# mrvollger/rustybam

Hardware: NVIDIA B200
Metric: lifted window-records/s (higher is better)
Workload: dtype u32/u64 (+f32 identities)

## Files before the change

rustybam_b200/csrc/rb_kernels.cu:

```cuda
#include <algorithm>
#include <cstdio>

#include "f32_fmt.cuh"
#include "lift_core.cuh"
#include "rb_kernels.cuh"
#include "rec_core.cuh"
#include "stream_core.cuh"

namespace rb {

__device__ __forceinline__ uint4 ld_nc_v4(const void* p) {
    uint4 r;
    asm volatile("ld.global.nc.L1::no_allocate.v4.u32 {%0,%1,%2,%3}, [%4];" : "=r"(r.x), "=r"(r.y), "=r"(r.z), "=r"(r.w) : "l"(p));
    return r;
}
__device__ __forceinline__ unsigned long long ld_volatile_u64(const unsigned long long* p) {
    unsigned long long v;
    asm volatile("ld.volatile.global.u64 %0, [%1];" : "=l"(v) : "l"(p));
    return v;
}
__device__ __forceinline__ uint32_t ld_volatile_u32(const uint32_t* p) {
    uint32_t v;
    asm volatile("ld.volatile.global.u32 %0, [%1];" : "=r"(v) : "l"(p));
    return v;
}
__device__ __forceinline__ uint4 ld_cg_v4(const void* p) {
    uint4 r;
    asm volatile("ld.global.cg.v4.u32 {%0,%1,%2,%3}, [%4];" : "=r"(r.x), "=r"(r.y), "=r"(r.z), "=r"(r.w) : "l"(p));
    return r;
}
__device__ __forceinline__ void report(unsigned long long* slot, uint64_t key, uint32_t code) {
    atomicMin(slot, (unsigned long long)((key << 8) | code));
}
__device__ __forceinline__ uint32_t nondigit_bytes(uint32_t x) {
    const uint32_t t = x ^ 0x30303030u;
    return (((t & 0x7F7F7F7Fu) + 0x76767676u) | t) & 0x80808080u;
}
__device__ __forceinline__ uint32_t nondigit_count(uint4 c) {
    return __popc(nondigit_bytes(c.x)) + __popc(nondigit_bytes(c.y)) + __popc(nondigit_bytes(c.z)) + __popc(nondigit_bytes(c.w));
}
// ... 50 lines not shown
    }
    if (lane == 0) atomicExch(&state[tile], LB_PRE | (excl + agg));
    return excl;
}

__device__ __forceinline__ void lb_publish(unsigned long long* state, uint64_t tile, unsigned long long agg) {
    atomicExch(&state[tile], (tile == 0 ? LB_PRE : LB_AGG) | agg);
}
__device__ __forceinline__ unsigned long long lb_walk(unsigned long long* state, uint64_t tile, unsigned long long agg) {
    const int lane = threadIdx.x & 31;
    if (tile == 0) return 0;
    unsigned long long excl = 0;
    long long look = (long long)tile - 1;
    for (;;) {
        const long long idx = look - lane;
        unsigned long long s = LB_PRE;
        if (idx >= 0) {
            s = ld_volatile_u64(&state[idx]);
            while ((s >> 62) == 0) { __nanosleep(64); s = ld_volatile_u64(&state[idx]); }
        }
        const unsigned pm = __ballot_sync(0xffffffffu, (s >> 62) == 2);
        const int first = pm ? (__ffs(pm) - 1) : 32;
        unsigned long long v = (lane <= first) ? (s & LB_VAL) : 0ull;
#pragma unroll
        for (int d = 16; d > 0; d >>= 1) v += __shfl_xor_sync(0xffffffffu, v, d);
        excl += v;
        if (pm) break;
        look -= 32;
    }
    if (lane == 0) atomicExch(&state[tile], LB_PRE | (excl + agg));
    return excl;
}

__device__ __noinline__ bool exact_len(const uint8_t* text, uint64_t pos, uint32_t& len, uint32_t& err) {
    long long s = (long long)pos;
    while (text[s - 1] >= '0' && text[s - 1] <= '9') s--;
    if (s == (long long)pos) { err = RE_CIGAR_PARSE; return false; }
    unsigned long long v = 0;
    for (long long k = s; k < (long long)pos; k++) {
        v = v * 10ull + (unsigned long long)(text[k] - '0');
        if (v > 0xFFFFFFFFull) { err = RE_CIGAR_PARSE; return false; }
    }
    if (v > MAX_OP_LEN) { err = RE_UNSUPPORTED; return false; }
    len = (uint32_t)v;
    return true;
}

__device__ __forceinline__ uint32_t smem_u32(const void* p) { return (uint32_t)__cvta_generic_to_shared(p); }
__device__ __forceinline__ void mbar_init(unsigned long long* bar, uint32_t count) {
    asm volatile("mbarrier.init.shared::cta.b64 [%0], %1;" ::"r"(smem_u32(bar)), "r"(count) : "memory");
    asm volatile("fence.mbarrier_init.release.cluster;" ::: "memory");
}
__device__ __forceinline__ void mbar_expect_tx(unsigned long long* bar, uint32_t bytes) {
    asm volatile("mbarrier.arrive.expect_tx.shared::cta.b64 _, [%0], %1;" ::"r"(smem_u32(bar)), "r"(bytes) : "memory");
}
__device__ __forceinline__ void bulk_g2s(void* dst, const void* src, uint32_t bytes, unsigned long long* bar) {
    asm volatile("cp.async.bulk.shared::cluster.global.mbarrier::complete_tx::bytes [%0], [%1], %2, [%3];" ::"r"(smem_u32(dst)),
                 "l"(src), "r"(bytes), "r"(smem_u32(bar))
                 : "memory");
}
__device__ __forceinline__ void fence_proxy_async() { asm volatile("fence.proxy.async.shared::cta;" ::: "memory"); }
__device__ __forceinline__ void bulk_s2g(void* dst, const void* src, uint32_t bytes) {
    asm volatile("cp.async.bulk.global.shared::cta.bulk_group [%0], [%1], %2;" ::"l"(dst), "r"(smem_u32(src)), "r"(bytes) : "memory");
    asm volatile("cp.async.bulk.commit_group;" ::: "memory");
}
__device__ __forceinline__ void bulk_wait_read() { asm volatile("cp.async.bulk.wait_group.read 0;" ::: "memory"); }
__device__ __forceinline__ void mbar_wait(unsigned long long* bar, uint32_t parity) {
    asm volatile(
        "{\n"
        ".reg .pred P1;\n"
        "LAB_WAIT:\n"
        "mbarrier.try_wait.parity.shared::cta.b64 P1, [%0], %1;\n"
        "@P1 bra DONE;\n"
        "bra LAB_WAIT;\n"
        "DONE:\n"
        "}\n" ::"r"(smem_u32(bar)),
        "r"(parity)
        : "memory");
}
__device__ __forceinline__ uint32_t parse4(uint32_t x) {
    x &= 0x0F0F0F0Fu;
    const uint32_t pairs = ((x * 2561u) >> 8) & 0x00FF00FFu;
    return (pairs * 6553601u) >> 16;
}

__global__ void __launch_bounds__(TOK_THREADS)
k_tokenise(const uint8_t* __restrict__ text, uint32_t* __restrict__ ops, unsigned long long* tile_state, unsigned int* ticket,
           ErrSlots err, uint32_t* misc_flags) {
    __shared__ __align__(16) uint8_t s_text[16 + TOK_TILE + 16];
    __shared__ uint16_t s_pos[TOK_TILE / 2];
#if RB_TOK_EARLY_PUBLISH
    __shared__ uint32_t s_opw[TOK_TILE / 2];
#endif
    __shared__ uint8_t s_lut[256];
    __shared__ __align__(8) unsigned long long s_bar;
    __shared__ uint32_t s_warp[TOK_THREADS / 32];
    __shared__ unsigned long long s_base;
    __shared__ unsigned int s_tile;

    const int tid = threadIdx.x, lane = tid & 31, warp = tid >> 5;
    if (tid < 256) s_lut[tid] = (uint8_t)code_of_char((uint32_t)tid);
    if (tid == 0) {
        s_tile = atomicAdd(ticket, 1u);
        mbar_init(&s_bar, 1);
    }
    __syncthreads();
    const uint64_t tile = s_tile;
    const uint64_t tbase = tile * (uint64_t)TOK_TILE;
    if (tid == 0) {
        mbar_expect_tx(&s_bar, 16 + TOK_TILE);
        bulk_g2s(s_text, text + tbase - 16, 16 + TOK_TILE, &s_bar);
    }
    mbar_wait(&s_bar, 0);

    const uint4 c = *reinterpret_cast<const uint4*>(s_text + 16 + tid * 16);
    const uint32_t M = 0x01020408u;
    const uint32_t m16 = ((((nondigit_bytes(c.x) >> 7) * M) >> 24) & 0xFu) | (((((nondigit_bytes(c.y) >> 7) * M) >> 24) & 0xFu) << 4) |
                         (((((nondigit_bytes(c.z) >> 7) * M) >> 24) & 0xFu) << 8) | (((((nondigit_bytes(c.w) >> 7) * M) >> 24) & 0xFu) << 12);
    const uint32_t cnt = __popc(m16);

    uint32_t inc = cnt;
#pragma unroll
    for (int d = 1; d < 32; d <<= 1) {
        const uint32_t t = __shfl_up_sync(0xffffffffu, inc, d);
        if (lane >= d) inc += t;
    }
    if (lane == 31) s_warp[warp] = inc;
    {
        uint32_t mm = m16, k = 0;
        const uint32_t wex = inc - cnt;
        __syncthreads();
        uint32_t wpre = 0, total = 0;
#pragma unroll
        for (int w = 0; w < TOK_THREADS / 32; w++) {
            const uint32_t t = s_warp[w];
            if (w < warp) wpre += t;
            total += t;
        }
#if RB_TOK_EARLY_PUBLISH
        if (tid == 0) lb_publish(tile_state, tile, total);
#else
        if (warp == 0) {
            const unsigned long long ex = lookback_u64(tile_state, tile, total);
            if (lane == 0) s_base = ex;
        }
#endif
        uint32_t idx = wpre + wex;
        while (mm) {
            const uint32_t j = __ffs(mm) - 1;
            mm &= mm - 1;
            s_pos[idx + k] = (uint16_t)(tid * 16 + j);
            k++;
        }
        __syncthreads();
        const uint32_t* s_w = reinterpret_cast<const uint32_t*>(s_text);
        uint32_t seen_codes = 0;
#if !RB_TOK_EARLY_PUBLISH
        const uint64_t base = s_base;
        uint32_t* out_ops = ops + base;
#endif
        for (uint32_t q = tid; q < total; q += TOK_THREADS) {
            const uint32_t e = s_pos[q];
            const uint32_t a = (e + 8) >> 2, sh = ((e + 8) & 3) * 8;
            const uint32_t w0 = s_w[a], w1 = s_w[a + 1], w2 = s_w[a + 2];
            uint32_t lo = __funnelshift_r(w0, w1, sh);
            uint32_t hi = __funnelshift_r(w1, w2, sh);
            uint32_t nd;
            if (q > 0) {
                nd = e - s_pos[q - 1] - 1u;
                nd = nd > 8u ? 8u : nd;
            } else {
                const uint32_t nh = nondigit_bytes(hi), nl = nondigit_bytes(lo);
                nd = nh ? (__clz(nh) >> 3) : (4u + (nl ? (__clz(nl) >> 3) : 4u));
            }
            const uint32_t code = s_lut[s_text[16 + e]];
            uint32_t len;
            if (nd - 1u >= 7u || code == 15u) {
                uint32_t ecode = RE_CIGAR_PARSE;
                len = 0;
                if (code == 15u || !exact_len(text, tbase + e, len, ecode)) { report(err.tok, tbase + e, ecode); len = 0; }
            } else {
                const unsigned long long x = (((unsigned long long)hi << 32) | lo) & (~0ull << (8u * (8u - nd)));
                len = parse4((uint32_t)(x >> 32));
                if (nd > 4u) len += parse4((uint32_t)x) * 10000u;
            }
            seen_codes |= 1u << code;
            const uint32_t word = (len << 4) | (code == 15u ? (uint32_t)OP_P : code);
#if RB_TOK_EARLY_PUBLISH
            s_opw[q] = word;
#else
            out_ops[q] = word;
#endif
        }
        const uint32_t seen_clip = seen_codes & ((1u << OP_S) | (1u << OP_H));
        if (seen_clip) atomicOr(misc_flags, 1u);
#if RB_TOK_EARLY_PUBLISH
        if (warp == 0) {
            const unsigned long long ex = lb_walk(tile_state, tile, total);
            if (lane == 0) s_base = ex;
        }
        __syncthreads();
        uint32_t* out_ops = ops + s_base;
        for (uint32_t q = tid; q < total; q += TOK_THREADS) out_ops[q] = s_opw[q];
#endif
    }
}

__global__ void __launch_bounds__(256)
k_rec_ops(const uint8_t* __restrict__ text, const uint64_t* __restrict__ cigar_off, uint32_t n_rec,
          const unsigned long long* __restrict__ tile_state, uint64_t* __restrict__ op_off, uint32_t* heads, ErrSlots err) {
    const uint32_t r = (blockIdx.x * blockDim.x + threadIdx.x) >> 5;
    const int lane = threadIdx.x & 31;
    if (r > n_rec) return;
    const uint64_t c = cigar_off[r];
    const uint64_t tile = c / TOK_TILE, tbase = tile * (uint64_t)TOK_TILE;
    const uint64_t prefix = tile ? (tile_state[tile - 1] & LB_VAL) : 0ull;
    const uint32_t nfull = (uint32_t)((c - tbase) >> 4), rem = (uint32_t)((c - tbase) & 15u);
    uint32_t cnt = 0;
    for (uint32_t j = lane; j < nfull; j += 32) cnt += nondigit_count(ld_nc_v4(text + tbase + (uint64_t)j * 16u));
    if (lane == 0 && rem) {
        const uint4 x = ld_nc_v4(text + tbase + (uint64_t)nfull * 16u);
        const uint32_t xw[4] = {x.x, x.y, x.z, x.w};
        for (uint32_t j = 0; j < rem; j++) cnt += ((((xw[j >> 2] >> ((j & 3) * 8)) & 0xFFu) - 48u) >= 10u);
    }
#pragma unroll
    for (int d = 16; d > 0; d >>= 1) cnt += __shfl_xor_sync(0xffffffffu, cnt, d);
    if (lane == 0) {
        const uint64_t o = prefix + cnt;
        op_off[r] = o;
        if (r < n_rec) {
            const uint64_t len = cigar_off[r + 1] - c;
            if (len > 0) {
                atomicOr(&heads[o >> 5], 1u << (o & 31u));
                const uint32_t last = text[c + len - 1], first = text[c];
                if ((last - 48u) < 10u) report(err.rec, r, RE_CIGAR_PARSE);
                if ((first - 48u) >= 10u) report(err.rec, r, RE_CIGAR_PARSE);
            }
        }
    }
}

__device__ __forceinline__ uint32_t flip_indel(uint32_t w) {
    const uint32_t c = op_code(w);
    return (c == OP_I || c == OP_D) ? (w ^ 3u) : w;
}
__global__ void __launch_bounds__(256)
k_invert_ops(uint32_t* __restrict__ ops, const uint64_t* __restrict__ op_off, uint32_t n_rec, const uint8_t* __restrict__ strand) {
    const uint64_t k = (uint64_t)blockIdx.x * blockDim.x + threadIdx.x;
    if (n_rec == 0 || k >= op_off[n_rec]) return;
    uint32_t lo = 0, hi = n_rec;
    while (lo < hi) {
        const uint32_t mid = lo + ((hi - lo) >> 1);
        if (op_off[mid] <= k) lo = mid + 1; else hi = mid;
    }
    const uint32_t r = lo - 1;
    const uint64_t a = op_off[r], b = op_off[r + 1];
    if (strand[r] != '-') { ops[k] = flip_indel(ops[k]); return; }
    const uint64_t i = k - a, m = b - 1 - i;
    if (k < m) {
        const uint32_t x = ops[k], y = ops[m];
        ops[k] = flip_indel(y);
// ... 589 lines not shown
#pragma unroll
        for (int k = 0; k < SMP_THREADS / 32; k++) btot = seg_combine(btot, s_warp[k]);
#if RB_SMP2_LB2
        const SegVal ex = lookback_seg2(blk_agg, b, btot);
#else
        const SegVal ex = lookback_seg(blk_state, blk_agg, blk_pre, b, btot);
#endif
        if (lane == 0) s_blk = ex;
    } else {
        for (int k = 0; k < warp; k++) wpre = seg_combine(wpre, s_warp[k]);
    }
    __syncthreads();
    SegVal pre = seg_combine(seg_combine(s_blk, wpre), exl);
    if (h & 1u) pre.c = ctr_zero();
    if (no_subs) pre.c.aux = (pre.c.aux & ~SUB_ABS) | SUB_ABS;
    if (nvalid) samples[chunk * SUBS] = pre.c;
}

constexpr uint32_t TS_NONE = 0xFFFFFFFFu;
__global__ void __launch_bounds__(256)
k_rec_heads(const uint8_t* __restrict__ text, const uint64_t* __restrict__ cigar_off, uint32_t n_rec, uint64_t* __restrict__ head_pos,
            uint32_t* tile_first) {
    const uint32_t r = blockIdx.x * blockDim.x + threadIdx.x;
    if (r >= n_rec) return;
    const uint64_t c = cigar_off[r], e = cigar_off[r + 1];
    uint64_t hp = ~0ull;
    const uint64_t lim = (e - c > 16u) ? c + 16u : e;
    for (uint64_t p = c; p < lim; p++)
        if (((uint32_t)text[p] - 48u) >= 10u) { hp = p; break; }
    head_pos[r] = hp;
    if (hp != ~0ull) atomicMin(&tile_first[hp / TOK_TILE], r);
}

#ifndef RB_TOKSCAN_MINB
#define RB_TOKSCAN_MINB 4
#endif
__global__ void __launch_bounds__(TOK_THREADS, RB_TOKSCAN_MINB)
k_tok_scan(const uint8_t* __restrict__ text, uint32_t* __restrict__ ops, unsigned long long* tile_state, unsigned int* ticket,
           ErrSlots err, uint32_t* misc_flags, const uint32_t* __restrict__ tile_first, const uint64_t* __restrict__ head_pos,
           uint32_t n_rec, Ctr* __restrict__ samples, uint32_t* seg_state, ScanPayload* seg_agg, ScanPayload* seg_pre) {
    __shared__ __align__(16) uint8_t s_text[16 + TOK_TILE + 16];
    __shared__ uint16_t s_pos[TOK_TILE / 2];
    __shared__ uint32_t s_opw[TOK_TILE / 2];
    __shared__ uint32_t s_head[TOK_TILE / 64 + 1];
    __shared__ uint16_t s_excl[TOK_THREADS], s_m16[TOK_THREADS];
    __shared__ uint8_t s_lut[256];
    __shared__ __align__(8) unsigned long long s_bar;
    __shared__ uint32_t s_warp[TOK_THREADS / 32];
    __shared__ SegVal s_wagg[TOK_THREADS / 32];
    __shared__ SegVal s_blk;
    __shared__ unsigned long long s_base;
    __shared__ unsigned int s_tile;
    __shared__ uint32_t s_prev0;

    const int tid = threadIdx.x, lane = tid & 31, warp = tid >> 5;
    if (tid < 256) s_lut[tid] = (uint8_t)code_of_char((uint32_t)tid);
    if (tid < TOK_TILE / 64 + 1) s_head[tid] = 0u;
    if (tid == 0) {
        s_tile = atomicAdd(ticket, 1u);
        mbar_init(&s_bar, 1);
        s_prev0 = 99u;
    }
    __syncthreads();
    const uint64_t tile = s_tile;
    const uint64_t tbase = tile * (uint64_t)TOK_TILE;
    if (tid == 0) {
        mbar_expect_tx(&s_bar, 16 + TOK_TILE);
        bulk_g2s(s_text, text + tbase - 16, 16 + TOK_TILE, &s_bar);
    }
    uint32_t r_first = TS_NONE;
    if (warp == TOK_THREADS / 32 - 1) r_first = tile_first[tile];
    mbar_wait(&s_bar, 0);

    const uint4 c = *reinterpret_cast<const uint4*>(s_text + 16 + tid * 16);
    const uint32_t M = 0x01020408u;
    const uint32_t m16 = ((((nondigit_bytes(c.x) >> 7) * M) >> 24) & 0xFu) | (((((nondigit_bytes(c.y) >> 7) * M) >> 24) & 0xFu) << 4) |
                         (((((nondigit_bytes(c.z) >> 7) * M) >> 24) & 0xFu) << 8) | (((((nondigit_bytes(c.w) >> 7) * M) >> 24) & 0xFu) << 12);
    const uint32_t cnt = __popc(m16);
    uint32_t inc = cnt;
#pragma unroll
    for (int d = 1; d < 32; d <<= 1) {
        const uint32_t t = __shfl_up_sync(0xffffffffu, inc, d);
        if (lane >= d) inc += t;
    }
    if (lane == 31) s_warp[warp] = inc;
    s_m16[tid] = (uint16_t)m16;
    __syncthreads();
    uint32_t wpre = 0, total = 0;
#pragma unroll
    for (int w = 0; w < TOK_THREADS / 32; w++) {
        const uint32_t t = s_warp[w];
        if (w < warp) wpre += t;
        total += t;
    }
    if (warp == 0) {
        const unsigned long long ex = lookback_u64(tile_state, tile, total);
        if (lane == 0) s_base = ex;
    }
    {
        uint32_t mm = m16, k = 0;
        const uint32_t idx = wpre + inc - cnt;
        s_excl[tid] = (uint16_t)idx;
        while (mm) {
            const uint32_t j = __ffs(mm) - 1;
            mm &= mm - 1;
            s_pos[idx + k] = (uint16_t)(tid * 16 + j);
            k++;
        }
    }
    __syncthreads();
    const uint64_t base = s_base;
    if (r_first != TS_NONE) {
        const uint64_t tend = tbase + TOK_TILE;
        for (uint64_t r = (uint64_t)r_first + lane; r < n_rec; r += 32) {
            const uint64_t hp = head_pos[r];
            if (hp == ~0ull) continue;
            if (hp >= tend) break;
            const uint32_t bpos = (uint32_t)(hp - tbase), t = bpos >> 4;
            const uint32_t j = (uint32_t)s_excl[t] + __popc((uint32_t)s_m16[t] & ((1u << (bpos & 15u)) - 1u));
            atomicOr(&s_head[j >> 5], 1u << (j & 31u));
        }
    }
    {
        const uint32_t* s_w = reinterpret_cast<const uint32_t*>(s_text);
        uint32_t seen_codes = 0;
        uint32_t* out_ops = ops + base;
        for (uint32_t q = tid; q < total; q += TOK_THREADS) {
            const uint32_t e = s_pos[q];
            const uint32_t a = (e + 8) >> 2, sh = ((e + 8) & 3) * 8;
            const uint32_t w0 = s_w[a], w1 = s_w[a + 1], w2 = s_w[a + 2];
            uint32_t lo = __funnelshift_r(w0, w1, sh);
            uint32_t hi = __funnelshift_r(w1, w2, sh);
            uint32_t nd;
            if (q > 0) {
                nd = e - s_pos[q - 1] - 1u;
                nd = nd > 8u ? 8u : nd;
            } else {
                const uint32_t nh = nondigit_bytes(hi), nl = nondigit_bytes(lo);
                nd = nh ? (__clz(nh) >> 3) : (4u + (nl ? (__clz(nl) >> 3) : 4u));
                int p = 16 + (int)e - 1;
                while (p >= 0 && ((uint32_t)s_text[p] - 48u) < 10u) p--;
                s_prev0 = (p >= 0) ? (uint32_t)s_lut[s_text[p]] : 99u;
            }
            const uint32_t code = s_lut[s_text[16 + e]];
            uint32_t len;
            if (nd - 1u >= 7u || code == 15u) {
                uint32_t ecode = RE_CIGAR_PARSE;
                len = 0;
                if (code == 15u || !exact_len(text, tbase + e, len, ecode)) { report(err.tok, tbase + e, ecode); len = 0; }
            } else {
                const unsigned long long x = (((unsigned long long)hi << 32) | lo) & (~0ull << (8u * (8u - nd)));
                len = parse4((uint32_t)(x >> 32));
                if (nd > 4u) len += parse4((uint32_t)x) * 10000u;
            }
            seen_codes |= 1u << code;
            const uint32_t word = (len << 4) | (code == 15u ? (uint32_t)OP_P : code);
            out_ops[q] = word;
            s_opw[q] = word;
        }
        const uint32_t seen_clip = seen_codes & ((1u << OP_S) | (1u << OP_H));
        if (seen_clip) atomicOr(misc_flags, 1u);
    }
    __syncthreads();

    const uint32_t off = (uint32_t)(base & 7u);
    const uint32_t ngroups = total ? ((total + off + 7u) >> 3) : 0u;
    const uint32_t per = (ngroups + TOK_THREADS - 1) / TOK_THREADS;
    const uint32_t g0 = (uint32_t)tid * per;
    const int lo_op = (int)(g0 * 8u) - (int)off;
    const uint32_t j_lo = lo_op < 0 ? 0u : (uint32_t)lo_op;
    uint32_t j_hi = (g0 + per) * 8u - off;
    j_hi = j_hi > total ? total : j_hi;
    SegVal mine = seg_identity();
    if (g0 < ngroups) {
        uint32_t slowc = 0;
        uint32_t prev_code = j_lo ? op_code(s_opw[j_lo - 1]) : s_prev0;
        for (uint32_t j = j_lo; j < j_hi; j++) {
            const uint32_t w = s_opw[j];
            const bool head = (s_head[j >> 5] >> (j & 31u)) & 1u;
            if (head) { mine.c = ctr_zero(); slowc = 0; mine.flag = 1u; }
            const uint32_t code = op_code(w), n = op_len(w);
            slowc += ((n - 1u) >= (ACC_BIG - 1u)) | ((!head) & (code == prev_code));
            ctr_add_op(mine.c, w);
            prev_code = code;
        }
        mine.c.aux = (mine.c.aux & AUX_OVF) | (slowc & AUX_CNT);
    }
    SegVal sinc = mine;
#pragma unroll
    for (int d = 1; d < 32; d <<= 1) {
        const SegVal y = seg_shfl(sinc, (lane - d) & 31);
        if (lane >= d) sinc = seg_combine(y, sinc);
    }
    if (lane == 31) s_wagg[warp] = sinc;
    SegVal exl = seg_shfl(sinc, (lane - 1) & 31);
    if (lane == 0) exl = seg_identity();
    __syncthreads();
    SegVal wp = seg_identity();
    if (warp == 0) {
        SegVal btot = seg_identity();
#pragma unroll
        for (int k = 0; k < TOK_THREADS / 32; k++) btot = seg_combine(btot, s_wagg[k]);
#ifdef RB_TS_NOLB
        const SegVal ex = btot;
#else
        const SegVal ex = lookback_seg(seg_state, seg_agg, seg_pre, tile, btot);
#endif
        if (lane == 0) s_blk = ex;
    } else {
        for (int k = 0; k < warp; k++) wp = seg_combine(wp, s_wagg[k]);
    }
    __syncthreads();
    if (g0 >= ngroups) return;
    SegVal pre = seg_combine(seg_combine(s_blk, wp), exl);
    for (uint32_t gi = 0; gi < per && g0 + gi < ngroups; gi++) {
        const int ls = (int)((g0 + gi) * 8u) - (int)off;
        if (gi) {
            const uint32_t a0 = (ls - 8) < 0 ? 0u : (uint32_t)(ls - 8);
            uint32_t slowc = pre.c.aux & AUX_CNT, ovf = pre.c.aux & AUX_OVF;
            uint32_t prev_code = a0 ? op_code(s_opw[a0 - 1]) : s_prev0;
            for (uint32_t j = a0; j < (uint32_t)ls; j++) {
                const uint32_t w = s_opw[j];
                const bool head = (s_head[j >> 5] >> (j & 31u)) & 1u;
                if (head) { pre.c = ctr_zero(); slowc = 0; ovf = 0; }
                const uint32_t code = op_code(w), n = op_len(w);
                slowc += ((n - 1u) >= (ACC_BIG - 1u)) | ((!head) & (code == prev_code));
                pre.c.aux = 0;
                ctr_add_op(pre.c, w);
                ovf |= pre.c.aux & AUX_OVF;
                prev_code = code;
            }
            pre.c.aux = ovf | (slowc & AUX_CNT);
        }
        if (ls < 0 || (uint32_t)ls >= total) continue;
        Ctr out = pre.c;
// ... 1700 lines not shown
    put_op(out_text + body_of(r) + pos, op_len(w), op_code(w));
}

static size_t samples2_smem() { return (size_t)(SMP_THREADS * SAMPLE + 9 * SMP_THREADS) * sizeof(uint32_t); }
static size_t scan_lift_smem(bool lift) {
    return (size_t)(SMP_THREADS * (SAMPLE + 1) + 9 * SMP_THREADS + (lift ? 2 * SL_WCAP : 0)) * sizeof(uint32_t);
}
int init_kernel_attrs() {
    cudaError_t e = cudaFuncSetAttribute(k_scan_lift<true>, cudaFuncAttributeMaxDynamicSharedMemorySize, (int)scan_lift_smem(true));
    if (e == cudaSuccess) e = cudaFuncSetAttribute(k_scan_lift<false>, cudaFuncAttributeMaxDynamicSharedMemorySize, (int)scan_lift_smem(false));
    if (e == cudaSuccess) e = cudaFuncSetAttribute(k_samples2<true>, cudaFuncAttributeMaxDynamicSharedMemorySize, (int)samples2_smem());
    if (e == cudaSuccess) e = cudaFuncSetAttribute(k_samples2<false>, cudaFuncAttributeMaxDynamicSharedMemorySize, (int)samples2_smem());
    if (e == cudaSuccess) e = cudaFuncSetAttribute(k_samples2<false, true>, cudaFuncAttributeMaxDynamicSharedMemorySize, (int)samples2_smem());
    if (e == cudaSuccess) e = cudaFuncSetAttribute(k_serialise, cudaFuncAttributeMaxDynamicSharedMemorySize, SER_CAP);
    if (e == cudaSuccess) e = cudaFuncSetAttribute(k_emit<false>, cudaFuncAttributeMaxDynamicSharedMemorySize, EMIT_DYN_BYTES);
    if (e == cudaSuccess) e = cudaFuncSetAttribute(k_emit<true>, cudaFuncAttributeMaxDynamicSharedMemorySize, EMIT_DYN_BYTES);
    return e == cudaSuccess ? 0 : -1;
}
__global__ void k_add_u64(unsigned long long* __restrict__ p, uint64_t n, unsigned long long delta) {
    const uint64_t i = (uint64_t)blockIdx.x * blockDim.x + threadIdx.x;
    if (i < n) p[i] += delta;
}
void launch_add_u64(uint64_t* p, uint64_t n, uint64_t delta, cudaStream_t s) {
    if (n == 0 || delta == 0) return;
    k_add_u64<<<(unsigned)((n + 255) / 256), 256, 0, s>>>(reinterpret_cast<unsigned long long*>(p), n, delta);
}
void launch_whole_text(const uint32_t* ops, const uint64_t* op_off, uint32_t n_rec, const RecInfo* recs, const Ctr* samples,
                       const uint64_t* line_off, uint8_t* out_text, uint64_t n_ops_bound, cudaStream_t s) {
    if (n_rec == 0 || n_ops_bound == 0 || out_text == nullptr) return;
    const uint64_t chunks = (n_ops_bound + SAMPLE - 1) / SAMPLE;
    k_whole_text<<<(unsigned)((chunks + WT_THREADS / 32 - 1) / (WT_THREADS / 32)), WT_THREADS, 0, s>>>(ops, op_off, n_rec, recs, samples,
                                                                                                    line_off, out_text);
}
void launch_tokenise(const uint8_t* text, uint64_t n_tiles, uint32_t* ops, unsigned long long* tile_state, unsigned int* ticket,
                     ErrSlots err, uint32_t* misc_flags, cudaStream_t s) {
    if (n_tiles == 0) return;
    k_tokenise<<<(unsigned)n_tiles, TOK_THREADS, 0, s>>>(text, ops, tile_state, ticket, err, misc_flags);
}
void launch_tok_scan(const uint8_t* text, uint64_t n_tiles, const uint64_t* cigar_off, uint32_t n_rec, uint32_t* ops,
                     unsigned long long* tile_state, unsigned int* ticket, ErrSlots err, uint32_t* misc_flags, uint32_t* tile_first,
                     uint64_t* head_pos, Ctr* samples, uint32_t* seg_state, ScanPayload* seg_agg, ScanPayload* seg_pre, cudaStream_t s) {
    if (n_tiles == 0) return;
    if (n_rec) k_rec_heads<<<(n_rec + 255) / 256, 256, 0, s>>>(text, cigar_off, n_rec, head_pos, tile_first);
    k_tok_scan<<<(unsigned)n_tiles, TOK_THREADS, 0, s>>>(text, ops, tile_state, ticket, err, misc_flags, tile_first, head_pos, n_rec,
                                                         samples, seg_state, seg_agg, seg_pre);
}
void launch_rec_ops(const uint8_t* text, const uint64_t* cigar_off, uint32_t n_rec, const unsigned long long* tile_state,
                    uint64_t* op_off, uint32_t* heads, ErrSlots err, cudaStream_t s) {
    const uint64_t warps = (uint64_t)n_rec + 1;
    k_rec_ops<<<(unsigned)((warps * 32 + 255) / 256), 256, 0, s>>>(text, cigar_off, n_rec, tile_state, op_off, heads, err);
}
void launch_scan_lift(bool lift, const uint32_t* ops, const uint64_t* n_ops_dev, uint64_t n_ops_bound, const uint32_t* heads,
                      Ctr* samples, uint32_t* blk_state, ScanPayload* blk_agg, ScanPayload* blk_pre, unsigned int* ticket,
                      LiftArgs la, cudaStream_t s, bool no_subs) {
    const uint64_t blocks = (n_ops_bound + SMP_OPS - 1) / SMP_OPS;
    if (blocks == 0) return;
    if (lift)
        k_scan_lift<true><<<(unsigned)blocks, SMP_THREADS, scan_lift_smem(true), s>>>(ops, n_ops_dev, heads, samples, blk_state, blk_agg,
                                                                                      blk_pre, ticket, la);
    else if (getenv("RB_OLD_SAMPLES"))
        k_scan_lift<false><<<(unsigned)blocks, SMP_THREADS, scan_lift_smem(false), s>>>(ops, n_ops_dev, heads, samples, blk_state,
                                                                                        blk_agg, blk_pre, ticket, la);
    else if (!getenv("RB_SAMPLES_LOCAL")) {
#if RB_SMP2_LB2
        cudaMemsetAsync(blk_agg, 0, blocks * sizeof(ScanPayload), s);
#endif
        if (no_subs)
            k_samples2<false, true><<<(unsigned)blocks, SMP_THREADS, samples2_smem(), s>>>(ops, n_ops_dev, heads, samples, blk_state, blk_agg, blk_pre,
                                                                                           ticket, 1u);
        else
            k_samples2<false><<<(unsigned)blocks, SMP_THREADS, samples2_smem(), s>>>(ops, n_ops_dev, heads, samples, blk_state, blk_agg, blk_pre, ticket,
                                                                                     0u);
    } else {
        k_samples2<true><<<(unsigned)blocks, SMP_THREADS, samples2_smem(), s>>>(ops, n_ops_dev, heads, samples, blk_state, blk_agg, blk_pre, ticket, 0u);
        k_blk_scan<<<1, 1024, 0, s>>>(n_ops_dev, blk_agg, blk_pre);
        const uint64_t chunks = (n_ops_bound + SAMPLE - 1) / SAMPLE;
        k_smp_fix<<<(unsigned)((chunks + 255) / 256), 256, 0, s>>>(n_ops_dev, blk_pre, samples);
// ... 213 lines not shown
```

rustybam_b200/csrc/rb_kernels.cuh:

```cuda
#pragma once
#include <cuda_runtime.h>

#include "lift_core.cuh"
#include "rb_common.cuh"
#include "trim_core.cuh"

namespace rb {

#ifndef RB_TOK_THREADS
#define RB_TOK_THREADS 256
#endif
constexpr int TOK_THREADS = RB_TOK_THREADS;
#ifndef RB_TOK_EARLY_PUBLISH
#define RB_TOK_EARLY_PUBLISH 1
#endif
constexpr int TOK_TILE = TOK_THREADS * 16;
constexpr int TEXT_FRONT_PAD = 16;
#ifndef RB_SMP_THREADS
#define RB_SMP_THREADS 256
#endif
constexpr int SMP_THREADS = RB_SMP_THREADS;
constexpr int SMP_OPS = SMP_THREADS * (int)SAMPLE;
constexpr int SL_WCAP = 2048;
#ifndef RB_LIFT_THREADS
#define RB_LIFT_THREADS 128
#endif
#ifndef RB_LIFT_CCAP
#define RB_LIFT_CCAP 96
#endif
#ifndef RB_LIFT_MINB
#define RB_LIFT_MINB 6
#endif
#ifndef RB_LIFT_STAGE_SMP
#define RB_LIFT_STAGE_SMP 1
#endif
#ifndef RB_LIFT_CHAIN
#define RB_LIFT_CHAIN 1
#endif
#ifndef RB_SMP2_LB2
#define RB_SMP2_LB2 0
#endif
#ifndef RB_SMP_MINB
#define RB_SMP_MINB 3
#endif
#ifndef RB_EMIT_MINB
#define RB_EMIT_MINB 6
#endif
#ifndef RB_EMIT_STAGE_TEXT
#define RB_EMIT_STAGE_TEXT 0
// ... 30 lines not shown
    const uint32_t* cont_hi;
    const uint32_t* pair_win;
    uint32_t general;
    uint32_t from_record;
};

struct RecInput {
    const uint64_t* cigar_off;
    const uint64_t *q_len, *q_st, *q_en, *t_len, *t_st, *t_en, *mapq;
    const uint8_t* strand;
    const uint32_t *q_id, *t_id;
    const uint64_t* names_off;
    const uint8_t* names;
    uint32_t n_rec;
    uint32_t no_text;
};

struct StatsDev {
    uint32_t *equal, *diff, *ins, *del, *ins_ev, *del_ev, *matches;
    float *id_m, *id_e, *id_a;
};
struct NumDev {
    uint64_t *q_st, *q_en, *t_st, *t_en, *nmatch, *aln_len;
    uint32_t *rec_idx, *win_idx;
};

struct ErrSlots {
    unsigned long long* tok;
    unsigned long long* rec;
};

int init_kernel_attrs();
void launch_add_u64(uint64_t* p, uint64_t n, uint64_t delta, cudaStream_t s);
void launch_tokenise(const uint8_t* text, uint64_t n_tiles, uint32_t* ops, unsigned long long* tile_state,
                     unsigned int* ticket, ErrSlots err, uint32_t* misc_flags, cudaStream_t s);
void launch_tok_scan(const uint8_t* text, uint64_t n_tiles, const uint64_t* cigar_off, uint32_t n_rec, uint32_t* ops,
                     unsigned long long* tile_state, unsigned int* ticket, ErrSlots err, uint32_t* misc_flags, uint32_t* tile_first,
                     uint64_t* head_pos, Ctr* samples, uint32_t* seg_state, ScanPayload* seg_agg, ScanPayload* seg_pre, cudaStream_t s);
void launch_rec_ops(const uint8_t* text, const uint64_t* cigar_off, uint32_t n_rec, const unsigned long long* tile_state,
                    uint64_t* op_off, uint32_t* heads, ErrSlots err, cudaStream_t s);
struct LiftArgs {
    const RecInfo* recs;
    const uint64_t* op_off;
    uint32_t n_rec;
    const uint32_t* rec_rank;
    const uint64_t* pair_off;
    const uint64_t* w_st;
    const uint64_t* w_en;
    HalfS* hs;
    HalfE* he;
};
void launch_scan_lift(bool lift, const uint32_t* ops, const uint64_t* n_ops_dev, uint64_t n_ops_bound, const uint32_t* heads,
                      Ctr* samples, uint32_t* blk_state, ScanPayload* blk_agg, ScanPayload* blk_pre, unsigned int* ticket,
                      LiftArgs la, cudaStream_t s, bool no_subs = false);
void launch_combine(uint64_t n_pairs, const uint64_t* pair_off, const uint32_t* rec_order, uint32_t n_rec, const RecInfo* recs,
                    const uint32_t* ops, WinView win, const uint64_t* names_off, const HalfS* hs, const HalfE* he, PairRes* res,
                    uint32_t* line_len, ErrSlots err, cudaStream_t s);
void launch_invert_ops(uint32_t* ops, const uint64_t* op_off, uint32_t n_rec, const uint8_t* strand, uint64_t n_ops_bound,
                       cudaStream_t s);
void launch_check_clips(const uint32_t* ops, const uint64_t* op_off, uint32_t n_rec, ErrSlots err, cudaStream_t s);
void launch_rec_prep(int mode, RecInput in, const uint64_t* op_off, const uint32_t* ops, const Ctr* samples, WinView win,
                     RecInfo* recs, uint32_t* pair_cnt, StatsDev st, ErrSlots err, cudaStream_t s);
void launch_pair_scan(const uint32_t* pair_cnt, const uint32_t* rec_order, uint32_t n_rec, uint64_t* pair_off, cudaStream_t s);
enum : uint32_t { PLAN_UNIFORM = 1u,
                  PLAN_FAST = 2u };
struct LiftPlan {
    uint32_t k0;
// ... 113 lines not shown
```

rustybam_b200/csrc/rbcuda.cu:

```cuda
#include <algorithm>
#include <chrono>
#include <condition_variable>
#include <cstdarg>
#include <cstdio>
#include <cstdlib>
#include <cstring>
#include <functional>
#include <mutex>
#include <string>
#include <thread>
#include <unordered_map>
#include <vector>

#include <sys/mman.h>

#include "../../include/rbcuda.h"
#include "name_intern.hpp"
#include "paf_parse_core.cuh"
#include "rb_kernels.cuh"
#include "rec_core.cuh"
#include "trim_rounds.hpp"

using namespace rb;

// ... 354 lines not shown
    NumDev d{};
    uint64_t* p = b->out_num.as<uint64_t>();
    d.q_st = p; d.q_en = p + n; d.t_st = p + 2 * n; d.t_en = p + 3 * n; d.nmatch = p + 4 * n; d.aln_len = p + 5 * n;
    d.rec_idx = reinterpret_cast<uint32_t*>(p + 6 * n);
    d.win_idx = d.rec_idx + n;
    return d;
}

bool tok_scan_enabled() {
    static const bool on = getenv("RB_TOKSCAN") != nullptr;
    return on;
}

int run_tok(rb_ctx* ctx, rb_batch* b) {
    cudaStream_t s = ctx->stream;
    uint32_t* sc = ctx->scalars.as<uint32_t>();
    CU(cudaMemsetAsync(sc, 0, 4 * sizeof(uint32_t), s));
    CU(cudaMemsetAsync(sc + SC_ERR_TOK, 0xFF, 4 * sizeof(uint32_t), s));
    CU(cudaMemsetAsync(b->tile_state.p, 0, b->n_tiles * 8, s));
    CU(cudaMemsetAsync(b->heads.p, 0, (b->ops_bound / SAMPLE + 2) * 4, s));
    CU(cudaMemsetAsync(b->blk_state.p, 0, (b->ops_bound / SMP_OPS + 2) * 4, s));
    ErrSlots err{reinterpret_cast<unsigned long long*>(sc + SC_ERR_TOK), reinterpret_cast<unsigned long long*>(sc + SC_ERR_REC)};
    const uint8_t* text = b->text_raw.as<uint8_t>() + TEXT_FRONT_PAD;
    b->have_samples = !b->invert && tok_scan_enabled();
    if (b->have_samples) {
        CU(cudaMemsetAsync(b->tile_first.p, 0xFF, b->n_tiles * 4, s));
        CU(cudaMemsetAsync(b->seg_state.p, 0, b->n_tiles * 4, s));
        KScope k(ctx, "k_tok_scan");
        launch_tok_scan(text, b->n_tiles, b->cigar_off.as<uint64_t>(), b->n_rec, b->ops.as<uint32_t>(), b->tile_state.as<unsigned long long>(),
                        sc + SC_TICKET_TOK, err, sc + SC_MISC, b->tile_first.as<uint32_t>(), b->head_pos.as<uint64_t>(), b->samples.as<Ctr>(),
                        b->seg_state.as<uint32_t>(), b->seg_agg.as<ScanPayload>(), b->seg_pre.as<ScanPayload>(), s);
    } else {
        KScope k(ctx, "k_tokenise");
        launch_tokenise(text, b->n_tiles, b->ops.as<uint32_t>(), b->tile_state.as<unsigned long long>(), sc + SC_TICKET_TOK, err,
                        sc + SC_MISC, s);
    }
    {
        KScope k(ctx, "k_rec_ops");
        launch_rec_ops(text, b->cigar_off.as<uint64_t>(), b->n_rec, b->tile_state.as<unsigned long long>(), b->op_off.as<uint64_t>(),
                       b->heads.as<uint32_t>(), err, s);
    }
    if (b->invert) {
        KScope k(ctx, "k_invert_ops");
        launch_invert_ops(b->ops.as<uint32_t>(), b->op_off.as<uint64_t>(), b->n_rec, b->strand.as<uint8_t>(), b->ops_bound, s);
    }
    CU(cudaGetLastError());
    return RB_OK;
}

int run_scan(rb_ctx* ctx, rb_batch* b, const LiftArgs* la, bool no_subs = false) {
    cudaStream_t s = ctx->stream;
    uint32_t* sc = ctx->scalars.as<uint32_t>();
    if (!la && b->have_samples) return RB_OK;
    {
        KScope k(ctx, la ? "k_scan_lift" : "k_samples");
        launch_scan_lift(la != nullptr, b->ops.as<uint32_t>(), b->op_off.as<uint64_t>() + b->n_rec, b->ops_bound, b->heads.as<uint32_t>(),
                         b->samples.as<Ctr>(), b->blk_state.as<uint32_t>(), b->blk_agg.as<ScanPayload>(), b->blk_pre.as<ScanPayload>(),
                         sc + SC_TICKET_SMP, la ? *la : LiftArgs{}, s, no_subs && !la);
    }
    CU(cudaGetLastError());
    return RB_OK;
}

}

extern "C" {

// ... 2603 lines not shown
```

Measured before the change: 447.6 million.

## Restructure CIGAR tokenizer to per-thread runs with staged vectorized op writes

The tokenise kernel now has each thread handle a 32-byte run instead of 16 bytes, which doubles the tile size. Each thread parses its own delimiters sequentially in registers instead of going through a shared position array and a second strided pass. Parsed words are staged in shared memory and written to global memory with aligned uint4 stores after the lookback. The k_tok_scan kernel is resized to keep its 16 bytes per thread under the larger tile, which changes its block size and min-blocks launch bound. A per-tile cap and a clamp on op_off are added to bound writes when the text ends early. The trade-off is more serial work per thread and fewer, larger tiles.

Result: faster. 478.8 million (median of 6 runs) (+7.0%).

```diff
diff --git a/rustybam_b200/csrc/rb_kernels.cu b/rustybam_b200/csrc/rb_kernels.cu
--- a/rustybam_b200/csrc/rb_kernels.cu
+++ b/rustybam_b200/csrc/rb_kernels.cu
@@ -6,6 +6,7 @@
 #include "rb_kernels.cuh"
 #include "rec_core.cuh"
 #include "stream_core.cuh"
+#include "tok_core.cuh"
 
 namespace rb {
 
@@ -122,18 +123,11 @@
     return excl;
 }
 
-__device__ __noinline__ bool exact_len(const uint8_t* text, uint64_t pos, uint32_t& len, uint32_t& err) {
-    long long s = (long long)pos;
-    while (text[s - 1] >= '0' && text[s - 1] <= '9') s--;
-    if (s == (long long)pos) { err = RE_CIGAR_PARSE; return false; }
-    unsigned long long v = 0;
-    for (long long k = s; k < (long long)pos; k++) {
-        v = v * 10ull + (unsigned long long)(text[k] - '0');
-        if (v > 0xFFFFFFFFull) { err = RE_CIGAR_PARSE; return false; }
-    }
-    if (v > MAX_OP_LEN) { err = RE_UNSUPPORTED; return false; }
-    len = (uint32_t)v;
-    return true;
+__device__ __noinline__ uint32_t tok_rare(const uint8_t* text, uint64_t pos, uint32_t code, unsigned long long* slot) {
+    uint32_t ecode;
+    const uint32_t w = tok_exact(text, pos, code, ecode);
+    if (ecode != RE_OK) report(slot, pos, ecode);
+    return w;
 }
 
 __device__ __forceinline__ uint32_t smem_u32(const void* p) { return (uint32_t)__cvta_generic_to_shared(p); }
@@ -175,13 +169,10 @@
 }
 
 __global__ void __launch_bounds__(TOK_THREADS)
-k_tokenise(const uint8_t* __restrict__ text, uint32_t* __restrict__ ops, unsigned long long* tile_state, unsigned int* ticket,
-           ErrSlots err, uint32_t* misc_flags) {
-    __shared__ __align__(16) uint8_t s_text[16 + TOK_TILE + 16];
-    __shared__ uint16_t s_pos[TOK_TILE / 2];
-#if RB_TOK_EARLY_PUBLISH
-    __shared__ uint32_t s_opw[TOK_TILE / 2];
-#endif
+k_tokenise(const uint8_t* __restrict__ text, uint64_t n_bytes, uint32_t* __restrict__ ops, unsigned long long* tile_state,
+           unsigned int* ticket, ErrSlots err, uint32_t* misc_flags) {
+    __shared__ __align__(16) uint8_t s_text[TOK_HALO + TOK_TILE];
+    __shared__ __align__(16) uint32_t s_opw[TOK_TILE / 2 + 4];
     __shared__ uint8_t s_lut[256];
     __shared__ __align__(8) unsigned long long s_bar;
     __shared__ uint32_t s_warp[TOK_THREADS / 32];
@@ -189,7 +180,7 @@
     __shared__ unsigned int s_tile;
 
     const int tid = threadIdx.x, lane = tid & 31, warp = tid >> 5;
-    if (tid < 256) s_lut[tid] = (uint8_t)code_of_char((uint32_t)tid);
+    for (int c = tid; c < 256; c += TOK_THREADS) s_lut[c] = (uint8_t)tok_code_of_char((uint32_t)c);
     if (tid == 0) {
         s_tile = atomicAdd(ticket, 1u);
         mbar_init(&s_bar, 1);
@@ -198,17 +189,20 @@
     const uint64_t tile = s_tile;
     const uint64_t tbase = tile * (uint64_t)TOK_TILE;
     if (tid == 0) {
-        mbar_expect_tx(&s_bar, 16 + TOK_TILE);
-        bulk_g2s(s_text, text + tbase - 16, 16 + TOK_TILE, &s_bar);
+        mbar_expect_tx(&s_bar, TOK_HALO + TOK_TILE);
+        bulk_g2s(s_text, text + tbase - TOK_HALO, TOK_HALO + TOK_TILE, &s_bar);
     }
     mbar_wait(&s_bar, 0);
 
-    const uint4 c = *reinterpret_cast<const uint4*>(s_text + 16 + tid * 16);
-    const uint32_t M = 0x01020408u;
-    const uint32_t m16 = ((((nondigit_bytes(c.x) >> 7) * M) >> 24) & 0xFu) | (((((nondigit_bytes(c.y) >> 7) * M) >> 24) & 0xFu) << 4) |
-                         (((((nondigit_bytes(c.z) >> 7) * M) >> 24) & 0xFu) << 8) | (((((nondigit_bytes(c.w) >> 7) * M) >> 24) & 0xFu) << 12);
-    const uint32_t cnt = __popc(m16);
-
+    const uint32_t* s_w = reinterpret_cast<const uint32_t*>(s_text);
+    uint32_t w[TOK_RUN / 4];
+#pragma unroll
+    for (int i = 0; i < TOK_RUN / 16; i++) {
+        const uint4 v = *reinterpret_cast<const uint4*>(s_text + TOK_HALO + tid * TOK_RUN + 16 * i);
+        w[4 * i] = v.x; w[4 * i + 1] = v.y; w[4 * i + 2] = v.z; w[4 * i + 3] = v.w;
+    }
+    const tok_mask_t<TOK_RUN> m = tok_run_mask<TOK_RUN>(w);
+    const uint32_t cnt = tok_popc(m);
     uint32_t inc = cnt;
 #pragma unroll
     for (int d = 1; d < 32; d <<= 1) {
@@ -216,84 +210,48 @@
         if (lane >= d) inc += t;
     }
     if (lane == 31) s_warp[warp] = inc;
-    {
-        uint32_t mm = m16, k = 0;
-        const uint32_t wex = inc - cnt;
-        __syncthreads();
-        uint32_t wpre = 0, total = 0;
-#pragma unroll
-        for (int w = 0; w < TOK_THREADS / 32; w++) {
-            const uint32_t t = s_warp[w];
-            if (w < warp) wpre += t;
-            total += t;
-        }
-#if RB_TOK_EARLY_PUBLISH
-        if (tid == 0) lb_publish(tile_state, tile, total);
-#else
-        if (warp == 0) {
-            const unsigned long long ex = lookback_u64(tile_state, tile, total);
-            if (lane == 0) s_base = ex;
-        }
-#endif
-        uint32_t idx = wpre + wex;
-        while (mm) {
-            const uint32_t j = __ffs(mm) - 1;
-            mm &= mm - 1;
-            s_pos[idx + k] = (uint16_t)(tid * 16 + j);
-            k++;
-        }
-        __syncthreads();
-        const uint32_t* s_w = reinterpret_cast<const uint32_t*>(s_text);
-        uint32_t seen_codes = 0;
-#if !RB_TOK_EARLY_PUBLISH
-        const uint64_t base = s_base;
-        uint32_t* out_ops = ops + base;
-#endif
-        for (uint32_t q = tid; q < total; q += TOK_THREADS) {
-            const uint32_t e = s_pos[q];
-            const uint32_t a = (e + 8) >> 2, sh = ((e + 8) & 3) * 8;
-            const uint32_t w0 = s_w[a], w1 = s_w[a + 1], w2 = s_w[a + 2];
-            uint32_t lo = __funnelshift_r(w0, w1, sh);
-            uint32_t hi = __funnelshift_r(w1, w2, sh);
-            uint32_t nd;
-            if (q > 0) {
-                nd = e - s_pos[q - 1] - 1u;
-                nd = nd > 8u ? 8u : nd;
-            } else {
-                const uint32_t nh = nondigit_bytes(hi), nl = nondigit_bytes(lo);
-                nd = nh ? (__clz(nh) >> 3) : (4u + (nl ? (__clz(nl) >> 3) : 4u));
-            }
-            const uint32_t code = s_lut[s_text[16 + e]];
-            uint32_t len;
-            if (nd - 1u >= 7u || code == 15u) {
-                uint32_t ecode = RE_CIGAR_PARSE;
-                len = 0;
-                if (code == 15u || !exact_len(text, tbase + e, len, ecode)) { report(err.tok, tbase + e, ecode); len = 0; }
-            } else {
-                const unsigned long long x = (((unsigned long long)hi << 32) | lo) & (~0ull << (8u * (8u - nd)));
-                len = parse4((uint32_t)(x >> 32));
-                if (nd > 4u) len += parse4((uint32_t)x) * 10000u;
-            }
-            seen_codes |= 1u << code;
-            const uint32_t word = (len << 4) | (code == 15u ? (uint32_t)OP_P : code);
-#if RB_TOK_EARLY_PUBLISH
-            s_opw[q] = word;
-#else
-            out_ops[q] = word;
-#endif
-        }
-        const uint32_t seen_clip = seen_codes & ((1u << OP_S) | (1u << OP_H));
-        if (seen_clip) atomicOr(misc_flags, 1u);
-#if RB_TOK_EARLY_PUBLISH
-        if (warp == 0) {
-            const unsigned long long ex = lb_walk(tile_state, tile, total);
-            if (lane == 0) s_base = ex;
-        }
-        __syncthreads();
-        uint32_t* out_ops = ops + s_base;
-        for (uint32_t q = tid; q < total; q += TOK_THREADS) out_ops[q] = s_opw[q];
-#endif
-    }
+    __syncthreads();
+    uint32_t idx = inc - cnt, total = 0;
+#pragma unroll
+    for (int k = 0; k < TOK_THREADS / 32; k++) {
+        const uint32_t t = s_warp[k];
+        if (k < warp) idx += t;
+        total += t;
+    }
+    const uint32_t cap = tok_tile_cap(n_bytes, tbase, TOK_TILE);
+    total = total < cap ? total : cap;
+    if (tid == 0) lb_publish(tile_state, tile, total);
+    const uint32_t seen = tok_run<TOK_RUN>(
+        s_w, s_lut, (uint32_t)tid, m,
+        [&](uint32_t word) {
+            if (idx < cap) s_opw[idx] = word;
+            idx++;
+        },
+        [&](uint32_t p, uint32_t code) { return tok_rare(text, tbase + p - TOK_HALO, code, err.tok); });
+    if (seen & ((1u << OP_S) | (1u << OP_H))) atomicOr(misc_flags, 1u);
+    if (warp == 0) {
+        const unsigned long long ex = lb_walk(tile_state, tile, total);
+        if (lane == 0) s_base = ex;
+    }
+    __syncthreads();
+    const uint64_t base = s_base;
+    uint32_t* out = ops + base;
+    const uint32_t head = min((uint32_t)(-base) & 3u, total), n4 = (total - head) >> 2;
+    const uint4* s4 = reinterpret_cast<const uint4*>(s_opw);
+    if ((uint32_t)tid < head) out[tid] = s_opw[tid];
+    for (uint32_t k = tid; k < n4; k += TOK_THREADS) {
+        const uint4 x = s4[k], y = s4[k + 1];
+        uint4 o;
+        switch (head) {
+            case 0: o = x; break;
+            case 1: o = make_uint4(x.y, x.z, x.w, y.x); break;
+            case 2: o = make_uint4(x.z, x.w, y.x, y.y); break;
+            default: o = make_uint4(x.w, y.x, y.y, y.z); break;
+        }
+        *reinterpret_cast<uint4*>(out + head + 4 * k) = o;
+    }
+    const uint32_t q = head + 4 * n4 + (uint32_t)tid;
+    if (q < total) out[q] = s_opw[q];
 }
 
 __global__ void __launch_bounds__(256)
@@ -304,7 +262,7 @@
     if (r > n_rec) return;
     const uint64_t c = cigar_off[r];
     const uint64_t tile = c / TOK_TILE, tbase = tile * (uint64_t)TOK_TILE;
-    const uint64_t prefix = tile ? (tile_state[tile - 1] & LB_VAL) : 0ull;
+    const uint64_t prefix = tile ? (tile_state[tile - 1] & LB_VAL) : 0ull, incl = tile_state[tile] & LB_VAL;
     const uint32_t nfull = (uint32_t)((c - tbase) >> 4), rem = (uint32_t)((c - tbase) & 15u);
     uint32_t cnt = 0;
     for (uint32_t j = lane; j < nfull; j += 32) cnt += nondigit_count(ld_nc_v4(text + tbase + (uint64_t)j * 16u));
@@ -316,7 +274,7 @@
 #pragma unroll
     for (int d = 16; d > 0; d >>= 1) cnt += __shfl_xor_sync(0xffffffffu, cnt, d);
     if (lane == 0) {
-        const uint64_t o = prefix + cnt;
+        const uint64_t o = min(prefix + cnt, incl);
         op_off[r] = o;
         if (r < n_rec) {
             const uint64_t len = cigar_off[r + 1] - c;
@@ -972,10 +930,11 @@
     if (hp != ~0ull) atomicMin(&tile_first[hp / TOK_TILE], r);
 }
 
+constexpr int TS_THREADS = TOK_TILE / 16;
 #ifndef RB_TOKSCAN_MINB
-#define RB_TOKSCAN_MINB 4
+#define RB_TOKSCAN_MINB (1024 / TS_THREADS)
 #endif
-__global__ void __launch_bounds__(TOK_THREADS, RB_TOKSCAN_MINB)
+__global__ void __launch_bounds__(TS_THREADS, RB_TOKSCAN_MINB)
 k_tok_scan(const uint8_t* __restrict__ text, uint32_t* __restrict__ ops, unsigned long long* tile_state, unsigned int* ticket,
            ErrSlots err, uint32_t* misc_flags, const uint32_t* __restrict__ tile_first, const uint64_t* __restrict__ head_pos,
            uint32_t n_rec, Ctr* __restrict__ samples, uint32_t* seg_state, ScanPayload* seg_agg, ScanPayload* seg_pre) {
@@ -983,18 +942,18 @@
     __shared__ uint16_t s_pos[TOK_TILE / 2];
     __shared__ uint32_t s_opw[TOK_TILE / 2];
     __shared__ uint32_t s_head[TOK_TILE / 64 + 1];
-    __shared__ uint16_t s_excl[TOK_THREADS], s_m16[TOK_THREADS];
+    __shared__ uint16_t s_excl[TS_THREADS], s_m16[TS_THREADS];
     __shared__ uint8_t s_lut[256];
     __shared__ __align__(8) unsigned long long s_bar;
-    __shared__ uint32_t s_warp[TOK_THREADS / 32];
-    __shared__ SegVal s_wagg[TOK_THREADS / 32];
+    __shared__ uint32_t s_warp[TS_THREADS / 32];
+    __shared__ SegVal s_wagg[TS_THREADS / 32];
     __shared__ SegVal s_blk;
     __shared__ unsigned long long s_base;
     __shared__ unsigned int s_tile;
     __shared__ uint32_t s_prev0;
 
     const int tid = threadIdx.x, lane = tid & 31, warp = tid >> 5;
-    if (tid < 256) s_lut[tid] = (uint8_t)code_of_char((uint32_t)tid);
+    for (int c = tid; c < 256; c += TS_THREADS) s_lut[c] = (uint8_t)code_of_char((uint32_t)c);
     if (tid < TOK_TILE / 64 + 1) s_head[tid] = 0u;
     if (tid == 0) {
         s_tile = atomicAdd(ticket, 1u);
@@ -1009,7 +968,7 @@
         bulk_g2s(s_text, text + tbase - 16, 16 + TOK_TILE, &s_bar);
     }
     uint32_t r_first = TS_NONE;
-    if (warp == TOK_THREADS / 32 - 1) r_first = tile_first[tile];
+    if (warp == TS_THREADS / 32 - 1) r_first = tile_first[tile];
     mbar_wait(&s_bar, 0);
 
     const uint4 c = *reinterpret_cast<const uint4*>(s_text + 16 + tid * 16);
@@ -1028,7 +987,7 @@
     __syncthreads();
     uint32_t wpre = 0, total = 0;
 #pragma unroll
-    for (int w = 0; w < TOK_THREADS / 32; w++) {
+    for (int w = 0; w < TS_THREADS / 32; w++) {
         const uint32_t t = s_warp[w];
         if (w < warp) wpre += t;
         total += t;
@@ -1065,7 +1024,7 @@
         const uint32_t* s_w = reinterpret_cast<const uint32_t*>(s_text);
         uint32_t seen_codes = 0;
         uint32_t* out_ops = ops + base;
-        for (uint32_t q = tid; q < total; q += TOK_THREADS) {
+        for (uint32_t q = tid; q < total; q += TS_THREADS) {
             const uint32_t e = s_pos[q];
             const uint32_t a = (e + 8) >> 2, sh = ((e + 8) & 3) * 8;
             const uint32_t w0 = s_w[a], w1 = s_w[a + 1], w2 = s_w[a + 2];
@@ -1083,18 +1042,16 @@
                 s_prev0 = (p >= 0) ? (uint32_t)s_lut[s_text[p]] : 99u;
             }
             const uint32_t code = s_lut[s_text[16 + e]];
-            uint32_t len;
+            uint32_t word;
             if (nd - 1u >= 7u || code == 15u) {
-                uint32_t ecode = RE_CIGAR_PARSE;
-                len = 0;
-                if (code == 15u || !exact_len(text, tbase + e, len, ecode)) { report(err.tok, tbase + e, ecode); len = 0; }
+                word = tok_rare(text, tbase + e, code, err.tok);
             } else {
                 const unsigned long long x = (((unsigned long long)hi << 32) | lo) & (~0ull << (8u * (8u - nd)));
-                len = parse4((uint32_t)(x >> 32));
+                uint32_t len = parse4((uint32_t)(x >> 32));
                 if (nd > 4u) len += parse4((uint32_t)x) * 10000u;
+                word = (len << 4) | code;
             }
             seen_codes |= 1u << code;
-            const uint32_t word = (len << 4) | (code == 15u ? (uint32_t)OP_P : code);
             out_ops[q] = word;
             s_opw[q] = word;
         }
@@ -1105,7 +1062,7 @@
 
     const uint32_t off = (uint32_t)(base & 7u);
     const uint32_t ngroups = total ? ((total + off + 7u) >> 3) : 0u;
-    const uint32_t per = (ngroups + TOK_THREADS - 1) / TOK_THREADS;
+    const uint32_t per = (ngroups + TS_THREADS - 1) / TS_THREADS;
     const uint32_t g0 = (uint32_t)tid * per;
     const int lo_op = (int)(g0 * 8u) - (int)off;
     const uint32_t j_lo = lo_op < 0 ? 0u : (uint32_t)lo_op;
@@ -1140,7 +1097,7 @@
     if (warp == 0) {
         SegVal btot = seg_identity();
 #pragma unroll
-        for (int k = 0; k < TOK_THREADS / 32; k++) btot = seg_combine(btot, s_wagg[k]);
+        for (int k = 0; k < TS_THREADS / 32; k++) btot = seg_combine(btot, s_wagg[k]);
 #ifdef RB_TS_NOLB
         const SegVal ex = btot;
 #else
@@ -2907,17 +2864,17 @@
     k_whole_text<<<(unsigned)((chunks + WT_THREADS / 32 - 1) / (WT_THREADS / 32)), WT_THREADS, 0, s>>>(ops, op_off, n_rec, recs, samples,
                                                                                                     line_off, out_text);
 }
-void launch_tokenise(const uint8_t* text, uint64_t n_tiles, uint32_t* ops, unsigned long long* tile_state, unsigned int* ticket,
-                     ErrSlots err, uint32_t* misc_flags, cudaStream_t s) {
+void launch_tokenise(const uint8_t* text, uint64_t n_bytes, uint64_t n_tiles, uint32_t* ops, unsigned long long* tile_state,
+                     unsigned int* ticket, ErrSlots err, uint32_t* misc_flags, cudaStream_t s) {
     if (n_tiles == 0) return;
-    k_tokenise<<<(unsigned)n_tiles, TOK_THREADS, 0, s>>>(text, ops, tile_state, ticket, err, misc_flags);
+    k_tokenise<<<(unsigned)n_tiles, TOK_THREADS, 0, s>>>(text, n_bytes, ops, tile_state, ticket, err, misc_flags);
 }
 void launch_tok_scan(const uint8_t* text, uint64_t n_tiles, const uint64_t* cigar_off, uint32_t n_rec, uint32_t* ops,
                      unsigned long long* tile_state, unsigned int* ticket, ErrSlots err, uint32_t* misc_flags, uint32_t* tile_first,
                      uint64_t* head_pos, Ctr* samples, uint32_t* seg_state, ScanPayload* seg_agg, ScanPayload* seg_pre, cudaStream_t s) {
     if (n_tiles == 0) return;
     if (n_rec) k_rec_heads<<<(n_rec + 255) / 256, 256, 0, s>>>(text, cigar_off, n_rec, head_pos, tile_first);
-    k_tok_scan<<<(unsigned)n_tiles, TOK_THREADS, 0, s>>>(text, ops, tile_state, ticket, err, misc_flags, tile_first, head_pos, n_rec,
+    k_tok_scan<<<(unsigned)n_tiles, TS_THREADS, 0, s>>>(text, ops, tile_state, ticket, err, misc_flags, tile_first, head_pos, n_rec,
                                                          samples, seg_state, seg_agg, seg_pre);
 }
 void launch_rec_ops(const uint8_t* text, const uint64_t* cigar_off, uint32_t n_rec, const unsigned long long* tile_state,
diff --git a/rustybam_b200/csrc/rb_kernels.cuh b/rustybam_b200/csrc/rb_kernels.cuh
--- a/rustybam_b200/csrc/rb_kernels.cuh
+++ b/rustybam_b200/csrc/rb_kernels.cuh
@@ -11,10 +11,11 @@
 #define RB_TOK_THREADS 256
 #endif
 constexpr int TOK_THREADS = RB_TOK_THREADS;
-#ifndef RB_TOK_EARLY_PUBLISH
-#define RB_TOK_EARLY_PUBLISH 1
-#endif
-constexpr int TOK_TILE = TOK_THREADS * 16;
+#ifndef RB_TOK_RUN
+#define RB_TOK_RUN 32
+#endif
+constexpr int TOK_RUN = RB_TOK_RUN;
+constexpr int TOK_TILE = TOK_THREADS * TOK_RUN;
 constexpr int TEXT_FRONT_PAD = 16;
 #ifndef RB_SMP_THREADS
 #define RB_SMP_THREADS 256
@@ -111,7 +112,7 @@
 
 int init_kernel_attrs();
 void launch_add_u64(uint64_t* p, uint64_t n, uint64_t delta, cudaStream_t s);
-void launch_tokenise(const uint8_t* text, uint64_t n_tiles, uint32_t* ops, unsigned long long* tile_state,
+void launch_tokenise(const uint8_t* text, uint64_t n_bytes, uint64_t n_tiles, uint32_t* ops, unsigned long long* tile_state,
                      unsigned int* ticket, ErrSlots err, uint32_t* misc_flags, cudaStream_t s);
 void launch_tok_scan(const uint8_t* text, uint64_t n_tiles, const uint64_t* cigar_off, uint32_t n_rec, uint32_t* ops,
                      unsigned long long* tile_state, unsigned int* ticket, ErrSlots err, uint32_t* misc_flags, uint32_t* tile_first,
diff --git a/rustybam_b200/csrc/rbcuda.cu b/rustybam_b200/csrc/rbcuda.cu
--- a/rustybam_b200/csrc/rbcuda.cu
+++ b/rustybam_b200/csrc/rbcuda.cu
@@ -410,7 +410,7 @@
                         b->seg_state.as<uint32_t>(), b->seg_agg.as<ScanPayload>(), b->seg_pre.as<ScanPayload>(), s);
     } else {
         KScope k(ctx, "k_tokenise");
-        launch_tokenise(text, b->n_tiles, b->ops.as<uint32_t>(), b->tile_state.as<unsigned long long>(), sc + SC_TICKET_TOK, err,
+        launch_tokenise(text, b->n_bytes, b->n_tiles, b->ops.as<uint32_t>(), b->tile_state.as<unsigned long long>(), sc + SC_TICKET_TOK, err,
                         sc + SC_MISC, s);
     }
     {
diff --git a/rustybam_b200/csrc/tok_core.cuh b/rustybam_b200/csrc/tok_core.cuh
--- /dev/null
+++ b/rustybam_b200/csrc/tok_core.cuh
@@ -0,0 +1,131 @@
+#pragma once
+#include <stdint.h>
+
+#include <type_traits>
+
+#include "rec_core.cuh"
+
+namespace rb {
+
+constexpr int TOK_HALO = 16;
+
+RB_HD uint32_t tok_popc(uint64_t x) {
+#ifdef __CUDA_ARCH__
+    return (uint32_t)__popcll(x);
+#else
+    return (uint32_t)__builtin_popcountll(x);
+#endif
+}
+RB_HD uint32_t tok_ffs0(uint64_t x) {
+#ifdef __CUDA_ARCH__
+    return (uint32_t)__ffsll((long long)x) - 1u;
+#else
+    return (uint32_t)__builtin_ctzll(x);
+#endif
+}
+RB_HD uint32_t tok_clz(uint32_t x) {
+#ifdef __CUDA_ARCH__
+    return (uint32_t)__clz(x);
+#else
+    return (uint32_t)__builtin_clz(x);
+#endif
+}
+RB_HD uint32_t tok_fshr(uint32_t lo, uint32_t hi, uint32_t sh) {
+#ifdef __CUDA_ARCH__
+    return __funnelshift_r(lo, hi, sh);
+#else
+    return sh ? (lo >> sh) | (hi << (32u - sh)) : lo;
+#endif
+}
+
+RB_HD uint32_t tok_nondigit_bytes(uint32_t x) {
+    const uint32_t t = x ^ 0x30303030u;
+    return (((t & 0x7F7F7F7Fu) + 0x76767676u) | t) & 0x80808080u;
+}
+RB_HD uint32_t tok_nondigit_nibble(uint32_t x) { return (tok_nondigit_bytes(x) * 0x00204081u) >> 28; }
+
+RB_HD uint32_t tok_parse4(uint32_t x) {
+    x &= 0x0F0F0F0Fu;
+    const uint32_t pairs = ((x * 2561u) >> 8) & 0x00FF00FFu;
+    return (pairs * 6553601u) >> 16;
+}
+
+RB_HD uint32_t tok_code_of_char(uint32_t ch) {
+    switch (ch) {
+        case 'M': return OP_M; case 'I': return OP_I; case 'D': return OP_D; case 'N': return OP_N; case 'S': return OP_S;
+        case 'H': return OP_H; case 'P': return OP_P; case '=': return OP_EQ; case 'X': return OP_X;
+        default: return 15u;
+    }
+}
+
+RB_HD uint32_t tok_exact(const uint8_t* text, uint64_t pos, uint32_t code, uint32_t& ecode) {
+    ecode = RE_CIGAR_PARSE;
+    if (code == 15u) return OP_P;
+    long long s = (long long)pos;
+    while ((uint32_t)text[s - 1] - 48u < 10u) s--;
+    if (s == (long long)pos) return code;
+    unsigned long long v = 0;
+    for (long long k = s; k < (long long)pos; k++) {
+        v = v * 10ull + (unsigned long long)(text[k] - '0');
+        if (v > 0xFFFFFFFFull) return code;
+    }
+    if (v > MAX_OP_LEN) { ecode = RE_UNSUPPORTED; return code; }
+    ecode = RE_OK;
+    return ((uint32_t)v << 4) | code;
+}
+
+template <int S>
+using tok_mask_t = typename std::conditional<(S > 32), uint64_t, uint32_t>::type;
+
+template <int S>
+RB_HD tok_mask_t<S> tok_run_mask(const uint32_t* w) {
+    static_assert(S % 16 == 0 && S <= 64, "a run is 16, 32 or 64 bytes");
+    tok_mask_t<S> m = 0;
+#pragma unroll
+    for (int i = 0; i < S / 4; i++) m |= (tok_mask_t<S>)tok_nondigit_nibble(w[i]) << (4 * i);
+    return m;
+}
+
+template <int S, class Put, class Rare>
+RB_HD uint32_t tok_run(const uint32_t* sw, const uint8_t* lut, uint32_t t, tok_mask_t<S> m, Put put, Rare rare) {
+    const uint32_t p0 = TOK_HALO + t * (uint32_t)S;
+    uint32_t prev;
+    {
+        const uint32_t nh = tok_nondigit_bytes(sw[p0 / 4 - 1]), nl = tok_nondigit_bytes(sw[p0 / 4 - 2]);
+        prev = p0 - 1u - (nh ? tok_clz(nh) >> 3 : 4u + (nl ? tok_clz(nl) >> 3 : 5u));
+    }
+    uint32_t seen = 0;
+    while (m) {
+        const uint32_t p = p0 + tok_ffs0(m);
+        m &= m - 1;
+        const uint32_t nd = p - prev - 1u;
+        prev = p;
+        const uint32_t q = p - 4u, a = q >> 2, sh = (q & 3u) * 8u;
+        const uint32_t wa = sw[a], wb = sw[a + 1];
+        const uint32_t code = lut[(wb >> sh) & 0xFFu];
+        uint32_t word;
+        if (code == 15u || nd - 1u >= 8u) {
+            word = rare(p, code);
+        } else {
+            uint32_t hi = tok_fshr(wa, wb, sh);
+            if (nd < 4u) hi &= 0xFFFFFFFFu << (32u - 8u * nd);
+            uint32_t len = tok_parse4(hi);
+            if (nd > 4u) {
+                uint32_t lo = tok_fshr(sw[a - 1], wa, sh);
+                if (nd < 8u) lo &= 0xFFFFFFFFu << (64u - 8u * nd);
+                len += tok_parse4(lo) * 10000u;
+            }
+            word = (len << 4) | code;
+        }
+        seen |= 1u << (word & 15u);
+        put(word);
+    }
+    return seen;
+}
+
+RB_HD uint32_t tok_tile_cap(uint64_t n_bytes, uint64_t tbase, uint32_t tile_bytes) {
+    const uint64_t real = n_bytes - tbase < tile_bytes ? n_bytes - tbase : tile_bytes;
+    return (uint32_t)((real + 1u) / 2u);
+}
+
+}
```
